# leabouffaut/DAS4Whales

Measured on AMD Instinct MI355X. Metric: channel-samples/sec through f-k filter + matched-filter, higher is better.
Workload: dtype f32 (matched filter: 2 x f16 split operands on the matrix cores, f32 accumulate); 1 GPU; 20000 channels x 120000 samples float32 per GPU, classic f-k fan mask (fk_filter_design defaults), stages fk+mf, HF+LF fin-call templates; api=public, parallelism=independent channel blocks x1

## Files before the change

das4whales_amd/csrc/xcorr_mm.hip:

```cpp
#include <cstdlib>

#include "mm_common.h"

namespace d4w {

#ifndef D4W_MM_CH
#define D4W_MM_CH 4096
#endif
constexpr int kMmCH = D4W_MM_CH;
constexpr int kMmKS = 6;
constexpr int kMmKSLong = 8;
constexpr int kMmKSMax = 16;
constexpr int kMmSection = 32 * kMmKSMax - 16;
constexpr int kMmMaxSupport = 32 * kMmKSLong - 15;
constexpr int kMmMaxSections = 16;
constexpr int kMmThreads = 256;
template <int KSM>
struct MmGeom {
    static constexpr int Halo = 32 * KSM;
    static constexpr int Stage = kMmCH + Halo;
    static constexpr int Q = (Stage + 4 * kMmThreads - 1) / (4 * kMmThreads);
    static constexpr int LastQ = (Stage - (Q - 1) * 4 * kMmThreads) / 4;
    static constexpr int Arr = Stage + 8;
};
__host__ __device__ constexpr int mm_pidx(int h) { return h; }

struct MmArgs {
    const float* x;
    const float* xnext;
    const double* mean;
    const float* maxabs;
    const float* taps;
    float* y0;
    float* y1;
    int nx, ns, ld_next, n_next, ltaps, len0, len1;
    float* rowmax0;
    float* rowmax1;
    int clamp;
    int shift;
    int accumulate;
    float tail0, tail1;
};

__device__ __forceinline__ float mm_wave_scan(float v) {
#ifdef D4W_EMU
    const int lane = (int)(threadIdx.x & 63);
    for (int off = 1; off < 64; off <<= 1) {
        const float n = __shfl_up(v, (unsigned)off);
        if (lane >= off) v += n;
    }
    return v;
#else
    auto dpp = [](float x, auto ctrl, auto rmask) {
        return __int_as_float(__builtin_amdgcn_update_dpp(0, __float_as_int(x), decltype(ctrl)::value, decltype(rmask)::value, 0xf, false));
    };
    v += dpp(v, std::integral_constant<int, 0x111>{}, std::integral_constant<int, 0xf>{});
    v += dpp(v, std::integral_constant<int, 0x112>{}, std::integral_constant<int, 0xf>{});
    v += dpp(v, std::integral_constant<int, 0x114>{}, std::integral_constant<int, 0xf>{});
    v += dpp(v, std::integral_constant<int, 0x118>{}, std::integral_constant<int, 0xf>{});
    v += dpp(v, std::integral_constant<int, 0x142>{}, std::integral_constant<int, 0xa>{});
    v += dpp(v, std::integral_constant<int, 0x143>{}, std::integral_constant<int, 0xc>{});
    return v;
#endif
}

template <int KS0, int KS1, int WPS, bool TAIL = false, bool WMAX = false, bool WSPLIT = false>
__global__ __launch_bounds__(kMmThreads, WPS) void xcorr_mm_rows(MmArgs P) {
    static_assert(!(WSPLIT && KS1 > 0), "the wave-split kernel is the one-template code run by two wave pairs");
    constexpr int KSM = KS0 > KS1 ? KS0 : KS1;
    using GEO = MmGeom<KSM>;
    constexpr int kMmHalo = GEO::Halo, kMmStage = GEO::Stage, kMmQ = GEO::Q, kMmLastQ = GEO::LastQ, kMmArr = GEO::Arr;
    constexpr int kSeg = 4 * kMmQ;
    D4W_DYN_LDS(smem_raw);
    mm_half* lds = reinterpret_cast<mm_half*>(smem_raw);
    float* red = reinterpret_cast<float*>(lds + 4 * kMmArr);
    constexpr int kBlk = kMmCH / 4;
    float* pb = red + 8;
    float* wt = pb + 2 * kBlk;
    const int tid = (int)threadIdx.x;
    const int lane = tid & 63, wv = mm_uniform(tid >> 6);
    const int n16 = lane & 15, g = lane >> 4;
    const int ns = P.ns;
    const int tsel = WSPLIT ? (wv >> 1) : 0;

    const int nchunk = (ns + kMmCH - 1) / kMmCH;
    const long long total = (long long)P.nx * nchunk;
    const int nparts = min(8, (int)gridDim.x);
    const int xcd = (int)blockIdx.x % nparts, wq = (int)blockIdx.x / nparts, nq = ((int)gridDim.x - xcd + nparts - 1) / nparts;
    const long long lo_c = total * xcd / nparts, hi_c = total * (xcd + 1) / nparts;
    mm_h8 a0h[KS0], a0l[KS0];
    mm_h8 a1h[KS1 ? KS1 : 1], a1l[KS1 ? KS1 : 1];
    float osc0 = 1.f, osc1 = 1.f;
#ifdef D4W_MM_V_TAIL_DEALT
    constexpr bool kRows = false;
#else
    constexpr bool kRows = TAIL;
#endif
    auto next_chunk = [&](long long c) -> long long {
        if constexpr (kRows) {
            const long long r = c / nchunk;
            return (c - r * nchunk + 1 < nchunk) ? c + 1 : (r + (long long)gridDim.x) * nchunk;
        } else {
            return c + nq;
        }
    };
    const long long end_c = kRows ? total : hi_c;
    long long c_n = kRows ? (long long)blockIdx.x * nchunk : lo_c + wq;
    {
        float* tl = reinterpret_cast<float*>(smem_raw);
        constexpr int TLP = 16 + kMmHalo;
        for (int i = tid; i < 2 * TLP; i += kMmThreads) {
            const int t = i / TLP, u = i - t * TLP - 15;
            const int L = t ? P.len1 : P.len0;
            float tv = (u >= 0 && u < L && (t == 0 || KS1 > 0 || WSPLIT)) ? P.taps[(size_t)t * P.ltaps + u] : 0.f;
            if constexpr (TAIL) {
                if (u < L && (t == 0 || KS1 > 0 || WSPLIT)) tv += t ? P.tail1 : P.tail0;
            }
            tl[i] = tv;
        }
        __syncthreads();
        auto build = [&](const float* tp, int L, auto& ah, auto& al, auto ks, float& osc) {
            constexpr int KS = decltype(ks)::value;
            float m = 0.f;
            for (int i = lane; i < TLP; i += 64) m = fmaxf(m, fabsf(tp[i]));
            for (int o = 32; o > 0; o >>= 1) m = fmaxf(m, __shfl_xor(m, o));
            float up, down;
            mm_pow2_scale(m, up, down);
            osc = up;
            (void)L;
            static_for<KS>([&](auto kq) {
                constexpr int kk = decltype(kq)::value;
                static_for<8>([&](auto jq) {
                    constexpr int j = decltype(jq)::value;
                    const float v = tp[15 + 32 * kk + 8 * g + j - n16] * down;
                    mm_half hi, lo;
                    mm_split(v, hi, lo);
                    mm_set(ah[kk], j, hi);
                    mm_set(al[kk], j, lo);
                });
            });
        };
        build(tl + (WSPLIT ? tsel * TLP : 0), WSPLIT && tsel ? P.len1 : P.len0, a0h, a0l, std::integral_constant<int, KS0>{}, osc0);
        if constexpr (KS1 > 0) build(tl + TLP, P.len1, a1h, a1l, std::integral_constant<int, KS1>{}, osc1);
        __syncthreads();
    }

    float4 pre[kMmQ];
    Mean2 mu_n{0.f, 0.f};
    float g_n = 1.f;
    bool heavy_n = false;
    bool tail_n = false;
    int row_n = 0, c0_n = 0;

    auto issue = [&](long long c) {
        row_n = (int)(c / nchunk);
        c0_n = (int)(c - (long long)row_n * nchunk) * kMmCH;
        mu_n = mean2_load(P.mean, row_n);
        g_n = 1.f;
        const int s0 = c0_n + P.shift;
        tail_n = s0 + kMmStage > ns;
        if (P.maxabs) {
            const float a = P.maxabs[row_n];
            g_n = (a > 0.f) ? 1.0f / a : 0.f;
            heavy_n = fabsf(mu_n.hi) > 0.9921875f * a;
        }
        const float* xr = P.x + (size_t)row_n * ns;
        const bool al = (reinterpret_cast<uintptr_t>(xr + s0) & 15) == 0;
        if (al && s0 + kMmStage <= ns) {
            const float4* p = reinterpret_cast<const float4*>(xr + s0) + tid;
            static_for<kMmQ>([&](auto qq) {
                constexpr int q = decltype(qq)::value;
                if (q < kMmQ - 1 || tid < kMmLastQ) pre[q] = mm_load4_stream(p + q * kMmThreads);
            });
        } else {
            if (al && (ns & 3) == 0) {
                static_for<kMmQ>([&](auto qq) {
                    constexpr int q = decltype(qq)::value;
                    if (q < kMmQ - 1 || tid < kMmLastQ) {
                        const int i = s0 + 4 * (tid + q * kMmThreads);
                        const float4 v = *reinterpret_cast<const float4*>(xr + min(i, ns - 4));
                        pre[q] = (i < ns) ? v : make_float4(mu_n.hi, mu_n.hi, mu_n.hi, mu_n.hi);
                    }
                });
            } else {
                static_for<kMmQ>([&](auto qq) {
                    constexpr int q = decltype(qq)::value;
                    if (q < kMmQ - 1 || tid < kMmLastQ) {
                        const int i = s0 + 4 * (tid + q * kMmThreads);
                        const float a0 = xr[min(i, ns - 1)], a1 = xr[min(i + 1, ns - 1)], a2 = xr[min(i + 2, ns - 1)], a3 = xr[min(i + 3, ns - 1)];
                        pre[q] = make_float4(i < ns ? a0 : mu_n.hi, i + 1 < ns ? a1 : mu_n.hi, i + 2 < ns ? a2 : mu_n.hi, i + 3 < ns ? a3 : mu_n.hi);
                    }
                });
            }
            if (P.xnext && P.n_next > 0 && s0 + kMmStage > ns) {
                const float* xn = P.xnext + (size_t)row_n * P.ld_next;
                const int n_next = P.n_next;
                static_for<kMmQ>([&](auto qq) {
                    constexpr int q = decltype(qq)::value;
                    if (q < kMmQ - 1 || tid < kMmLastQ) {
                        const int d = s0 + 4 * (tid + q * kMmThreads) - ns;
                        const float b0 = xn[min(max(d, 0), n_next - 1)], b1 = xn[min(max(d + 1, 0), n_next - 1)];
                        const float b2 = xn[min(max(d + 2, 0), n_next - 1)], b3 = xn[min(max(d + 3, 0), n_next - 1)];
                        if (d >= 0 && d < n_next) pre[q].x = b0;
                        if (d + 1 >= 0 && d + 1 < n_next) pre[q].y = b1;
                        if (d + 2 >= 0 && d + 2 < n_next) pre[q].z = b2;
                        if (d + 3 >= 0 && d + 3 < n_next) pre[q].w = b3;
                    }
                });
            }
        }
    };

    if (c_n < end_c) issue(c_n);
    int buf = 0;
    constexpr bool want_max = WMAX;
    float pst_hi = 0.f, pst_lo = 0.f;
    for (long long c = c_n; c < end_c;) {
        const int row = row_n, c0 = c0_n;
        const Mean2 mu = mu_n;
        const bool tail = tail_n;
        const int n_valid = ns + ((P.xnext && P.n_next > 0) ? P.n_next : 0) - c0 - P.shift;
        float gsc = g_n, osx = 1.f;
        const float gout = g_n;
        const bool own_scale = !P.maxabs || heavy_n;
        mm_half* bh = lds + (size_t)buf * 2 * kMmArr;
        mm_half* bl = bh + kMmArr;
        const long long c_next = next_chunk(c);
        const int cin = c0 / kMmCH;
        if (TAIL && cin == 0) { pst_hi = 0.f; pst_lo = 0.f; }
        const float pst = pst_hi;
        if (own_scale) {
            float m = 0.f;
            static_for<kMmQ>([&](auto qq) {
                constexpr int q = decltype(qq)::value;
                if (q < kMmQ - 1 || tid < kMmLastQ) {
                    const float4 v = pre[q];
                    const int at = 4 * (tid + q * kMmThreads);
                    float d0 = demean(v.x, mu), d1 = demean(v.y, mu), d2 = demean(v.z, mu), d3 = demean(v.w, mu);
                    if (tail) {
                        if (at >= n_valid) d0 = 0.f;
                        if (at + 1 >= n_valid) d1 = 0.f;
                        if (at + 2 >= n_valid) d2 = 0.f;
                        if (at + 3 >= n_valid) d3 = 0.f;
                    }
                    m = fmaxf(fmaxf(m, fmaxf(fabsf(d0), fabsf(d1))), fmaxf(fabsf(d2), fabsf(d3)));
                }
            });
            for (int o = 32; o > 0; o >>= 1) m = fmaxf(m, __shfl_xor(m, o));
            if (lane == 0) red[wv + 4 * buf] = m;
            lds_barrier();
            m = fmaxf(fmaxf(red[4 * buf], red[4 * buf + 1]), fmaxf(red[4 * buf + 2], red[4 * buf + 3]));
            mm_pow2_scale(m, osx, gsc);
        }
        const float mlg = -mu.lo * gsc;
        static_for<kMmQ>([&](auto qq) {
            constexpr int q = decltype(qq)::value;
            float s[4] = {0.f, 0.f, 0.f, 0.f};
            const bool mine = q < kMmQ - 1 || tid < kMmLastQ;
            const int at = mm_pidx(4 * (tid + q * kMmThreads));
            if (mine) {
                const float4 v = pre[q];
#ifdef D4W_MM_V_FLOATMEAN
                s[0] = (v.x - mu.hi) * gsc; s[1] = (v.y - mu.hi) * gsc; s[2] = (v.z - mu.hi) * gsc; s[3] = (v.w - mu.hi) * gsc;
#else
                s[0] = fmaf(v.x - mu.hi, gsc, mlg); s[1] = fmaf(v.y - mu.hi, gsc, mlg); s[2] = fmaf(v.z - mu.hi, gsc, mlg); s[3] = fmaf(v.w - mu.hi, gsc, mlg);
#endif
                if (P.clamp && !own_scale) static_for<4>([&](auto ee) { constexpr int e = decltype(ee)::value; s[e] = mm_clamp_half(s[e]); });
                if (tail) {
                    const int a0 = 4 * (tid + q * kMmThreads);
                    static_for<4>([&](auto ee) { constexpr int e = decltype(ee)::value; if (a0 + e >= n_valid) s[e] = 0.f; });
                }
#ifdef D4W_MM_V_OLDSPLIT
                mm_half h[4], l[4];
                static_for<4>([&](auto ee) { constexpr int e = decltype(ee)::value; mm_split(s[e], h[e], l[e]); });
                mm_put4(bh + at, h);
                mm_put4(bl + at, l);
#else
                mm_split_put4(s, bh + at, bl + at);
#endif
            }
#ifdef D4W_MM_V_TAIL_NOSCAN
            if constexpr (false) {
#else
            if constexpr (TAIL && q < kMmCH / (4 * kMmThreads)) {
#endif
                const float t4 = (s[0] + s[1]) + (s[2] + s[3]);
                const float inc = mm_wave_scan(t4);
                pb[buf * kBlk + kMmThreads * q + tid] = inc - t4;
                if (lane == 63) wt[buf * 16 + 4 * q + wv] = inc;
            }
        });
        if (c_next < end_c) issue(c_next);
        lds_barrier();
        float* ya = ((WSPLIT && tsel) ? P.y1 : P.y0) + (size_t)row * ns;
        float* yb = KS1 ? P.y1 + (size_t)row * ns : nullptr;
        const bool valign = ((reinterpret_cast<uintptr_t>(ya + c0) & 15) == 0) && (!KS1 || (reinterpret_cast<uintptr_t>(yb + c0) & 15) == 0);
        const float oxs = (own_scale && P.maxabs) ? osx * gout : osx;
        const float o0 = osc0 * oxs, o1 = osc1 * oxs;
        float segoff = 0.f;
        constexpr int NTW = kMmCH / 256 / (WSPLIT ? 2 : 4), NST = NTW * KSM, PF = 2;
        auto tile_of = [&](int ti) { return WSPLIT ? (wv & 1) + 2 * ti : wv + 4 * ti; };
        auto frag = [&](const mm_half* arr, int T, int kk) -> mm_h8 {
            const int gr = 32 * T + 2 * n16 + g + 4 * kk;
            return *reinterpret_cast<const mm_h8*>(arr + mm_pidx(8 * gr));
        };
        mm_h8 fh[PF + 1], fl[PF + 1];
        static_for<PF>([&](auto ss) {
            constexpr int s_ = decltype(ss)::value;
            fh[s_] = frag(bh, tile_of(s_ / KSM), s_ % KSM);
            fl[s_] = frag(bl, tile_of(s_ / KSM), s_ % KSM);
        });
        mm_f4 c0h = mm_zero(), c0l = mm_zero(), c1h = mm_zero(), c1l = mm_zero();
        float vmax0 = -INFINITY, vmax1 = -INFINITY;
        float vsum = 0.f;
        static_for<NST>([&](auto ss) {
            constexpr int s_ = decltype(ss)::value, ti = s_ / KSM, kk = s_ % KSM;
            if constexpr (s_ + PF < NST) {
                fh[(s_ + PF) % (PF + 1)] = frag(bh, tile_of((s_ + PF) / KSM), (s_ + PF) % KSM);
                fl[(s_ + PF) % (PF + 1)] = frag(bl, tile_of((s_ + PF) / KSM), (s_ + PF) % KSM);
            }
            mm_sched_fence();
            const mm_h8 xh = fh[s_ % (PF + 1)], xl = fl[s_ % (PF + 1)];
            if constexpr (kk < KS0) {
                c0h = mm_mfma(a0h[kk], xh, c0h);
                c0l = mm_mfma(a0h[kk], xl, c0l);
            }
            if constexpr (kk < KS1) {
                c1h = mm_mfma(a1h[kk], xh, c1h);
                c1l = mm_mfma(a1h[kk], xl, c1l);
            }
            if constexpr (kk < KS0) c0l = mm_mfma(a0l[kk], xh, c0l);
            if constexpr (kk < KS1) c1l = mm_mfma(a1l[kk], xh, c1l);
            mm_sched_fence();
            if constexpr (kk == KSM - 1) {
                const int T = tile_of(ti);
                const int kl = 256 * T + 16 * n16 + 4 * g;
                const int k = c0 + kl;
                if constexpr (ti == 0) {
                if constexpr (TAIL) {
                    const float w = lane < 16 ? wt[buf * 16 + lane] : 0.f;
                    const float inc = mm_wave_scan(w);
                    segoff = inc - w;
        #ifdef D4W_EMU
                    const float own = __shfl(inc, 15);
        #else
                    const float own = __builtin_bit_cast(float, __builtin_amdgcn_readlane(__builtin_bit_cast(int, inc), 15));
        #endif
                    const double pd = ((double)pst_hi + (double)pst_lo) + (double)(own * oxs);
                    const float ph = (float)pd, pl2 = (float)(pd - (double)ph);
        #ifdef D4W_EMU
                    pst_hi = ph; pst_lo = pl2;
        #else
                    pst_hi = __builtin_bit_cast(float, __builtin_amdgcn_readfirstlane(__builtin_bit_cast(int, ph)));
                    pst_lo = __builtin_bit_cast(float, __builtin_amdgcn_readfirstlane(__builtin_bit_cast(int, pl2)));
        #endif
                }
                }
                float r0[4], r1[4];
                float a0 = 0.f, a1 = 0.f;
#ifdef D4W_MM_V_TAIL_NOSCAN
                if constexpr (false) {
#else
                if constexpr (TAIL) {
#endif
#ifdef D4W_EMU
                    const float so = __shfl(segoff, T);
#else
                    const float so = __builtin_bit_cast(float, __builtin_amdgcn_readlane(__builtin_bit_cast(int, segoff), T));
#endif
                    const float pbk = fmaf(so + pb[buf * kBlk + kMmThreads * (T >> 2) + 64 * (T & 3) + 4 * n16], oxs, pst);
                    a0 = ((WSPLIT && tsel) ? P.tail1 : P.tail0) * pbk;
                    a1 = P.tail1 * pbk;
                }
                static_for<4>([&](auto rr) {
                    constexpr int r = decltype(rr)::value;
                    r0[r] = fmaf(fmaf(mm_get(c0l, r), kMmLoInv, mm_get(c0h, r)), o0, a0);
                    if constexpr (KS1 > 0) r1[r] = fmaf(fmaf(mm_get(c1l, r), kMmLoInv, mm_get(c1h, r)), o1, a1);
                });
                c0h = mm_zero(); c0l = mm_zero(); c1h = mm_zero(); c1l = mm_zero();
                if (valign && k + 3 < ns) {
                    if (KS1 == 0 && P.accumulate) {
                        const float4 o = mm_load4_stream(reinterpret_cast<const float4*>(ya + k));
                        r0[0] += o.x; r0[1] += o.y; r0[2] += o.z; r0[3] += o.w;
                    }
                    mm_store4(ya + k, r0[0], r0[1], r0[2], r0[3]);
                    if constexpr (KS1 > 0) mm_store4(yb + k, r1[0], r1[1], r1[2], r1[3]);
                    if (want_max) {
                        vmax0 = fmaxf(vmax0, fmaxf(fmaxf(r0[0], r0[1]), fmaxf(r0[2], r0[3])));
#ifndef D4W_MM_V_NONAN
                        vsum += (r0[0] + r0[1]) + (r0[2] + r0[3]);
#endif
                        if constexpr (KS1 > 0) {
                            vmax1 = fmaxf(vmax1, fmaxf(fmaxf(r1[0], r1[1]), fmaxf(r1[2], r1[3])));
#ifndef D4W_MM_V_NONAN
                            vsum += (r1[0] + r1[1]) + (r1[2] + r1[3]);
#endif
                        }
                    }
                } else {
                    for (int r = 0; r < 4; ++r)
                        if (k + r < ns) {
                            const float v0 = (KS1 == 0 && P.accumulate) ? ya[k + r] + r0[r] : r0[r];
                            ya[k + r] = v0;
                            if constexpr (KS1 > 0) yb[k + r] = r1[r];
                            if (want_max) {
                                vmax0 = fmaxf(vmax0, v0);
                                vsum += v0;
                                if constexpr (KS1 > 0) { vmax1 = fmaxf(vmax1, r1[r]); vsum += r1[r]; }
                            }
                        }
                }
            }
        });
        if (want_max) {
            for (int o = 32; o > 0; o >>= 1) {
                vmax0 = fmaxf(vmax0, __shfl_xor(vmax0, o));
                if constexpr (KS1 > 0) vmax1 = fmaxf(vmax1, __shfl_xor(vmax1, o));
            }
            const bool bad = __any(vsum != vsum);
            if (lane == 0) {
                mm_atomic_fmax(((WSPLIT && tsel) ? P.rowmax1 : P.rowmax0) + row, bad ? __uint_as_float(0x7FC00000u) : vmax0);
                if constexpr (KS1 > 0) mm_atomic_fmax(P.rowmax1 + row, bad ? __uint_as_float(0x7FC00000u) : vmax1);
            }
        }
        buf ^= 1;
        c = c_next;
    }
}

}

using namespace d4w;

extern "C" {

int d4w_xcorr_mm_max_support(void) { return kMmSection * kMmMaxSections; }

#define D4W_MM_LAUNCH(KS0, KS1, WPS, TAIL, grid, lds, stream, Q)                                                              \
    do {                                                                                                                      \
        if ((Q).rowmax0) D4W_LAUNCH((xcorr_mm_rows<KS0, KS1, WPS, TAIL, true>), dim3(grid), dim3(kMmThreads), lds, stream, Q);  \
        else D4W_LAUNCH((xcorr_mm_rows<KS0, KS1, WPS, TAIL, false>), dim3(grid), dim3(kMmThreads), lds, stream, Q);             \
    } while (0)

static int mm_one_template(MmArgs P, const float* taps, int len, float* y, float* rowmax, int grid, void* stream) {
    auto lds_of = [](int arr) { return (size_t)4 * arr * sizeof(mm_half) + 8 * sizeof(float); };
    const int nsec = (len <= 32 * kMmKSMax - 15) ? 1 : ceil_div(len, kMmSection);
    const int per = (nsec == 1) ? len : 16 * ceil_div(ceil_div(len, nsec), 16);
    for (int j = 0; j < nsec; ++j) {
        const int first = j * per;
        MmArgs Q = P;
        Q.taps = taps + first;
        Q.len0 = Q.len1 = std::min(per, len - first);
        Q.y0 = y;
        Q.y1 = nullptr;
        Q.shift = first;
        Q.accumulate = j > 0;
        Q.rowmax0 = (j == nsec - 1) ? rowmax : nullptr;
        Q.rowmax1 = nullptr;
        const int ks = ceil_div(Q.len0 + 15, 32);
        if (ks <= kMmKS)
            D4W_MM_LAUNCH(kMmKS, 0, 3, false, grid, lds_of(MmGeom<kMmKS>::Arr), stream, Q);
        else if (ks <= kMmKSLong)
            D4W_MM_LAUNCH(kMmKSLong, 0, 2, false, grid, lds_of(MmGeom<kMmKSLong>::Arr), stream, Q);
        else if (ks <= 12)
            D4W_MM_LAUNCH(12, 0, 2, false, grid, lds_of(MmGeom<12>::Arr), stream, Q);
        else
            D4W_MM_LAUNCH(kMmKSMax, 0, 2, false, grid, lds_of(MmGeom<kMmKSMax>::Arr), stream, Q);
    }
    return D4W_OK;
}

int d4w_xcorr_mm_f32(const float* x, int nx, int ns, const float* xnext, int ld_next, int n_next, const double* mean,
                     const float* maxabs, const float* taps, int ntpl, int ltaps, int len0, int len1, float* y0, float* y1,
                     void* stream) {
    return d4w_xcorr_mm_rowmax_f32(x, nx, ns, xnext, ld_next, n_next, mean, maxabs, taps, ntpl, ltaps, len0, len1, y0, y1, nullptr,
                                   nullptr, stream);
}

int d4w_xcorr_mm_rowmax_f32(const float* x, int nx, int ns, const float* xnext, int ld_next, int n_next, const double* mean,
                            const float* maxabs, const float* taps, int ntpl, int ltaps, int len0, int len1, float* y0, float* y1,
                            float* rowmax0, float* rowmax1, void* stream) {
    return d4w_xcorr_mm_tail_f32(x, nx, ns, xnext, ld_next, n_next, mean, maxabs, taps, ntpl, ltaps, len0, len1, 0.0, 0.0, y0, y1,
                                 rowmax0, rowmax1, stream);
}

int d4w_xcorr_mm_tail_max_support(void) { return 32 * kMmKSMax - 15; }

int d4w_xcorr_mm_tail_f32(const float* x, int nx, int ns, const float* xnext, int ld_next, int n_next, const double* mean,
                          const float* maxabs, const float* taps, int ntpl, int ltaps, int len0, int len1, double tail0, double tail1,
                          float* y0, float* y1, float* rowmax0, float* rowmax1, void* stream) {
    if (!x || !y0 || !taps || nx < 1 || ns < 1) return fail(D4W_EINVAL, "bad argument");
    if (ntpl == 2 && ((rowmax0 == nullptr) != (rowmax1 == nullptr))) return fail(D4W_EINVAL, "rowmax0 and rowmax1 go together");
    if (ntpl < 1 || ntpl > 2 || (ntpl == 2 && !y1)) return fail(D4W_EINVAL, "ntpl = %d (1 or 2 templates per call)", ntpl);
    if (xnext && (n_next < 0 || ld_next < n_next)) return fail(D4W_EINVAL, "a continuation needs 0 <= n_next <= ld_next");
    if (ntpl == 1) { len1 = len0; tail1 = 0.0; }
    if (len0 < 1 || len1 < 1 || len0 > ltaps || len1 > ltaps || std::max(len0, len1) > d4w_xcorr_mm_max_support())
        return fail(D4W_EINVAL, "template supports (%d, %d) must lie in 1..min(ltaps = %d, %d)", len0, len1, ltaps, d4w_xcorr_mm_max_support());
    const bool tails = tail0 != 0.0 || tail1 != 0.0;
    if (tails) {
        if (!mean || !maxabs) return fail(D4W_EINVAL, "the zero-padded template's tail needs the rows' statistics (mean, maxabs)");
        if (std::max(len0, len1) > d4w_xcorr_mm_tail_max_support())
            return fail(D4W_EINVAL, "with a tail the supports (%d, %d) must be <= %d", len0, len1, d4w_xcorr_mm_tail_max_support());
    }
    MmArgs P;
    P.x = x; P.xnext = xnext; P.mean = mean; P.maxabs = maxabs; P.taps = taps; P.y0 = y0; P.y1 = y1;
    P.nx = nx; P.ns = ns; P.ld_next = ld_next; P.n_next = xnext ? n_next : 0; P.ltaps = ltaps; P.len0 = len0; P.len1 = len1;
    P.shift = 0; P.accumulate = 0;
    static const int env_clamp = [] { const char* v = getenv("D4W_MM_CLAMP"); return v ? atoi(v) : 0; }();
    P.clamp = (xnext != nullptr && n_next > 0) || env_clamp;
    P.rowmax0 = rowmax0; P.rowmax1 = (ntpl == 2) ? rowmax1 : nullptr;
    P.tail0 = (float)tail0; P.tail1 = (float)tail1;
    if (rowmax0) {
        D4W_HIP(hipMemsetD32Async((hipDeviceptr_t)rowmax0, (int)0xFF800000u, (size_t)nx, (hipStream_t)stream));
        if (ntpl == 2) D4W_HIP(hipMemsetD32Async((hipDeviceptr_t)rowmax1, (int)0xFF800000u, (size_t)nx, (hipStream_t)stream));
    }
    const int nchunk = ceil_div(ns, kMmCH);
    const long long total = (long long)nx * nchunk;
    static const int env_wgs = [] { const char* v = getenv("D4W_MM_WGS"); const int n = v ? atoi(v) : 0; return n < 0 ? 0 : (n > 8 ? 8 : n); }();
    const int ks0 = ceil_div(len0 + 15, 32), ks1 = ceil_div(len1 + 15, 32);
    const bool fused = ntpl == 2 && std::max(ks0, ks1) <= kMmKS;
    const int per_cu = env_wgs ? env_wgs : ((ntpl == 1 && ks0 <= kMmKS) ? 3 : 2);
    const int ncu = mm_num_cus();
    const int grid = (int)std::min<long long>(total, (long long)ncu * per_cu);
    auto lds_of = [](int arr, bool tl) {
        return (size_t)4 * arr * sizeof(mm_half) + 8 * sizeof(float) + (tl ? ((size_t)2 * (kMmCH / 4) + 2 * 16) * sizeof(float) : 0);
    };
    static const int fused_form = [] { const char* v = getenv("D4W_MM_FUSED"); return v ? atoi(v) : 2; }();
    const int per_cu_ws = env_wgs ? env_wgs : 3;
#define D4W_MM_LAUNCH_WS(TAIL, grid, lds, Q)                                                                                            \
    do {                                                                                                                                \
        if ((Q).rowmax0) D4W_LAUNCH((xcorr_mm_rows<kMmKS, 0, 3, TAIL, true, true>), dim3(grid), dim3(kMmThreads), lds, stream, Q);       \
        else D4W_LAUNCH((xcorr_mm_rows<kMmKS, 0, 3, TAIL, false, true>), dim3(grid), dim3(kMmThreads), lds, stream, Q);                  \
    } while (0)
    if (tails) {
        const int grid_t = (int)std::min<long long>((long long)nx, (long long)ncu * per_cu);
        if (fused && fused_form != 2) {
            D4W_MM_LAUNCH_WS(true, (int)std::min<long long>((long long)nx, (long long)ncu * per_cu_ws), lds_of(MmGeom<kMmKS>::Arr, true), P);
            return D4W_OK;
        }
        if (fused) {
            const size_t lds = lds_of(MmGeom<kMmKS>::Arr, true);
            if (ks0 <= 5)
                D4W_MM_LAUNCH(5, kMmKS, 2, true, grid_t, lds, stream, P);
            else
                D4W_MM_LAUNCH(kMmKS, kMmKS, 2, true, grid_t, lds, stream, P);
            return D4W_OK;
        }
        for (int t = 0; t < ntpl; ++t) {
            MmArgs Q = P;
            Q.taps = taps + (size_t)t * ltaps;
            Q.len0 = Q.len1 = t ? len1 : len0;
            Q.tail0 = t ? (float)tail1 : (float)tail0;
            Q.tail1 = 0.f;
            Q.y0 = t ? y1 : y0;
            Q.y1 = nullptr;
            Q.rowmax0 = t ? rowmax1 : rowmax0;
            Q.rowmax1 = nullptr;
            const int ks = ceil_div(Q.len0 + 15, 32);
            if (ks <= kMmKS) {
                if (Q.rowmax0)
                    D4W_LAUNCH((xcorr_mm_rows<kMmKS, 0, 2, true, true>), dim3(grid_t), dim3(kMmThreads), lds_of(MmGeom<kMmKS>::Arr, true), stream, Q);
                else
                    D4W_LAUNCH((xcorr_mm_rows<kMmKS, 0, 3, true, false>), dim3(grid_t), dim3(kMmThreads), lds_of(MmGeom<kMmKS>::Arr, true), stream, Q);
            }
            else if (ks <= kMmKSLong)
                D4W_MM_LAUNCH(kMmKSLong, 0, 2, true, grid_t, lds_of(MmGeom<kMmKSLong>::Arr, true), stream, Q);
            else if (ks <= 12)
                D4W_MM_LAUNCH(12, 0, 2, true, grid_t, lds_of(MmGeom<12>::Arr, true), stream, Q);
            else
                D4W_MM_LAUNCH(kMmKSMax, 0, 2, true, grid_t, lds_of(MmGeom<kMmKSMax>::Arr, true), stream, Q);
        }
        return D4W_OK;
    }
    if (!fused) {
        int rc = mm_one_template(P, taps, len0, y0, rowmax0, grid, stream);
        if (rc == D4W_OK && ntpl == 2) rc = mm_one_template(P, taps + ltaps, len1, y1, rowmax1, grid, stream);
        return rc;
    }
    const size_t lds = lds_of(MmGeom<kMmKS>::Arr, false);
    if (fused_form != 2) {
        D4W_MM_LAUNCH_WS(false, (int)std::min<long long>(total, (long long)ncu * per_cu_ws), lds, P);
        return D4W_OK;
    }
    if (ks0 <= 5)
        D4W_MM_LAUNCH(5, kMmKS, 2, false, grid, lds, stream, P);
    else
        D4W_MM_LAUNCH(kMmKS, kMmKS, 2, false, grid, lds, stream, P);
    return D4W_OK;
}

}
```

Measured before the change: 119.1 billion channel-samples/s.

## Compute tail-correction prefix sums with MFMA ones-matrix and DPP row scans

Reworks the TAIL path's running-sum correction. It no longer does a full wave scan per float4 group and stores per-thread prefix values in LDS. Instead, each lane folds four group sums through quad-swap and row-shift DPP into 16-sample partials written to a small LDS table. The within-tile prefix is now obtained from an extra MFMA against a ones fragment plus a 16-lane row scan. This shrinks the LDS footprint and removes scattered LDS reads in the output epilogue, at the cost of one extra pair of MFMAs per tile and more DPP work.

```diff
diff --git a/das4whales_amd/csrc/xcorr_mm.hip b/das4whales_amd/csrc/xcorr_mm.hip
--- a/das4whales_amd/csrc/xcorr_mm.hip
+++ b/das4whales_amd/csrc/xcorr_mm.hip
@@ -42,6 +42,41 @@
     float tail0, tail1;
 };
 
+#ifndef D4W_EMU
+template <int CTRL, int RMASK = 0xf>
+__device__ __forceinline__ float mm_dpp(float v) {
+    return __int_as_float(__builtin_amdgcn_update_dpp(0, __float_as_int(v), CTRL, RMASK, 0xf, false));
+}
+#endif
+
+template <int N>
+__device__ __forceinline__ float mm_row_shr(float v) {
+#ifdef D4W_EMU
+    const float n = __shfl_up(v, (unsigned)N);
+    return ((int)(threadIdx.x & 15) >= N) ? n : 0.f;
+#else
+    return mm_dpp<0x110 + N>(v);
+#endif
+}
+
+template <int X>
+__device__ __forceinline__ float mm_quad_xor(float v) {
+    static_assert(X == 1 || X == 2, "a swap inside the quad");
+#ifdef D4W_EMU
+    return __shfl_xor(v, X);
+#else
+    return mm_dpp<X == 1 ? 0xB1 : 0x4E>(v);
+#endif
+}
+
+__device__ __forceinline__ float mm_row_scan(float v) {
+    v += mm_row_shr<1>(v);
+    v += mm_row_shr<2>(v);
+    v += mm_row_shr<4>(v);
+    v += mm_row_shr<8>(v);
+    return v;
+}
+
 __device__ __forceinline__ float mm_wave_scan(float v) {
 #ifdef D4W_EMU
     const int lane = (int)(threadIdx.x & 63);
@@ -51,16 +86,18 @@
     }
     return v;
 #else
-    auto dpp = [](float x, auto ctrl, auto rmask) {
-        return __int_as_float(__builtin_amdgcn_update_dpp(0, __float_as_int(x), decltype(ctrl)::value, decltype(rmask)::value, 0xf, false));
-    };
-    v += dpp(v, std::integral_constant<int, 0x111>{}, std::integral_constant<int, 0xf>{});
-    v += dpp(v, std::integral_constant<int, 0x112>{}, std::integral_constant<int, 0xf>{});
-    v += dpp(v, std::integral_constant<int, 0x114>{}, std::integral_constant<int, 0xf>{});
-    v += dpp(v, std::integral_constant<int, 0x118>{}, std::integral_constant<int, 0xf>{});
-    v += dpp(v, std::integral_constant<int, 0x142>{}, std::integral_constant<int, 0xa>{});
-    v += dpp(v, std::integral_constant<int, 0x143>{}, std::integral_constant<int, 0xc>{});
+    v = mm_row_scan(v);
+    v += mm_dpp<0x142, 0xa>(v);
+    v += mm_dpp<0x143, 0xc>(v);
     return v;
+#endif
+}
+
+__device__ __forceinline__ float mm_lane(float v, int L) {
+#ifdef D4W_EMU
+    return __shfl(v, L);
+#else
+    return __builtin_bit_cast(float, __builtin_amdgcn_readlane(__builtin_bit_cast(int, v), L));
 #endif
 }
 
@@ -74,9 +111,11 @@
     D4W_DYN_LDS(smem_raw);
     mm_half* lds = reinterpret_cast<mm_half*>(smem_raw);
     float* red = reinterpret_cast<float*>(lds + 4 * kMmArr);
-    constexpr int kBlk = kMmCH / 4;
-    float* pb = red + 8;
-    float* wt = pb + 2 * kBlk;
+    constexpr int kOwnQ = kMmCH / (4 * kMmThreads);
+    constexpr int kPart = kMmCH / 64;
+    constexpr int kPPL = kPart / 64;
+    static_assert(!TAIL || (kOwnQ % 4 == 0 && kPPL >= 1), "the tail's partial sums fold four loads into one value per lane");
+    float* wt = red + 8;
     const int tid = (int)threadIdx.x;
     const int lane = tid & 63, wv = mm_uniform(tid >> 6);
     const int n16 = lane & 15, g = lane >> 4;
@@ -95,6 +134,11 @@
     constexpr bool kRows = false;
 #else
     constexpr bool kRows = TAIL;
+#endif
+#ifdef D4W_MM_V_TAIL_NOSCAN
+    constexpr bool kTailSum = false;
+#else
+    constexpr bool kTailSum = TAIL;
 #endif
     auto next_chunk = [&](long long c) -> long long {
         if constexpr (kRows) {
@@ -144,6 +188,12 @@
         if constexpr (KS1 > 0) build(tl + TLP, P.len1, a1h, a1l, std::integral_constant<int, KS1>{}, osc1);
         __syncthreads();
     }
+    mm_h8 one_h, one_l;
+    static_for<8>([&](auto jq) {
+        constexpr int j = decltype(jq)::value;
+        mm_set(one_h, j, mm_to_half(g < 2 ? 1.f : 0.f));
+        mm_set(one_l, j, mm_to_half(g < 2 ? kMmLoInv : 0.f));
+    });
 
     float4 pre[kMmQ];
     Mean2 mu_n{0.f, 0.f};
@@ -253,6 +303,7 @@
             mm_pow2_scale(m, osx, gsc);
         }
         const float mlg = -mu.lo * gsc;
+        float t4[kOwnQ];
         static_for<kMmQ>([&](auto qq) {
             constexpr int q = decltype(qq)::value;
             float s[4] = {0.f, 0.f, 0.f, 0.f};
@@ -279,19 +330,24 @@
                 mm_split_put4(s, bh + at, bl + at);
 #endif
             }
-#ifdef D4W_MM_V_TAIL_NOSCAN
-            if constexpr (false) {
-#else
-            if constexpr (TAIL && q < kMmCH / (4 * kMmThreads)) {
-#endif
-                const float t4 = (s[0] + s[1]) + (s[2] + s[3]);
-                const float inc = mm_wave_scan(t4);
-                pb[buf * kBlk + kMmThreads * q + tid] = inc - t4;
-                if (lane == 63) wt[buf * 16 + 4 * q + wv] = inc;
-            }
+            if constexpr (kTailSum && q < kOwnQ) t4[q] = (s[0] + s[1]) + (s[2] + s[3]);
         });
+        if constexpr (kTailSum) {
+            const bool odd1 = (lane & 1) != 0, odd2 = (lane & 2) != 0;
+            static_for<kOwnQ / 4>([&](auto qg) {
+                constexpr int q0 = 4 * decltype(qg)::value;
+                const float m01 = (odd1 ? t4[q0 + 1] : t4[q0]) + mm_quad_xor<1>(odd1 ? t4[q0] : t4[q0 + 1]);
+                const float m23 = (odd1 ? t4[q0 + 3] : t4[q0 + 2]) + mm_quad_xor<1>(odd1 ? t4[q0 + 2] : t4[q0 + 3]);
+                float m = (odd2 ? m23 : m01) + mm_quad_xor<2>(odd2 ? m01 : m23);
+                m += mm_row_shr<4>(m);
+                m += mm_row_shr<8>(m);
+                if ((lane & 12) == 12) wt[buf * kPart + 16 * (q0 + (lane & 3)) + 4 * wv + g] = m;
+            });
+        }
         if (c_next < end_c) issue(c_next);
+#ifndef D4W_MM_V_NOHANDOFF
         lds_barrier();
+#endif
         float* ya = ((WSPLIT && tsel) ? P.y1 : P.y0) + (size_t)row * ns;
         float* yb = KS1 ? P.y1 + (size_t)row * ns : nullptr;
         const bool valign = ((reinterpret_cast<uintptr_t>(ya + c0) & 15) == 0) && (!KS1 || (reinterpret_cast<uintptr_t>(yb + c0) & 15) == 0);
@@ -311,6 +367,7 @@
             fl[s_] = frag(bl, tile_of(s_ / KSM), s_ % KSM);
         });
         mm_f4 c0h = mm_zero(), c0l = mm_zero(), c1h = mm_zero(), c1l = mm_zero();
+        mm_f4 cs = mm_zero();
         float vmax0 = -INFINITY, vmax1 = -INFINITY;
         float vsum = 0.f;
         static_for<NST>([&](auto ss) {
@@ -331,6 +388,7 @@
             }
             if constexpr (kk < KS0) c0l = mm_mfma(a0l[kk], xh, c0l);
             if constexpr (kk < KS1) c1l = mm_mfma(a1l[kk], xh, c1l);
+            if constexpr (kTailSum && kk == 0) cs = mm_mfma(one_l, xl, mm_mfma(one_h, xh, mm_zero()));
             mm_sched_fence();
             if constexpr (kk == KSM - 1) {
                 const int T = tile_of(ti);
@@ -338,14 +396,11 @@
                 const int k = c0 + kl;
                 if constexpr (ti == 0) {
                 if constexpr (TAIL) {
-                    const float w = lane < 16 ? wt[buf * 16 + lane] : 0.f;
+                    float w = 0.f;
+                    static_for<kPPL>([&](auto pp) { w += wt[buf * kPart + kPPL * lane + decltype(pp)::value]; });
                     const float inc = mm_wave_scan(w);
                     segoff = inc - w;
-        #ifdef D4W_EMU
-                    const float own = __shfl(inc, 15);
-        #else
-                    const float own = __builtin_bit_cast(float, __builtin_amdgcn_readlane(__builtin_bit_cast(int, inc), 15));
-        #endif
+                    const float own = mm_lane(inc, 63);
                     const double pd = ((double)pst_hi + (double)pst_lo) + (double)(own * oxs);
                     const float ph = (float)pd, pl2 = (float)(pd - (double)ph);
         #ifdef D4W_EMU
@@ -358,17 +413,10 @@
                 }
                 float r0[4], r1[4];
                 float a0 = 0.f, a1 = 0.f;
-#ifdef D4W_MM_V_TAIL_NOSCAN
-                if constexpr (false) {
-#else
-                if constexpr (TAIL) {
-#endif
-#ifdef D4W_EMU
-                    const float so = __shfl(segoff, T);
-#else
-                    const float so = __builtin_bit_cast(float, __builtin_amdgcn_readlane(__builtin_bit_cast(int, segoff), T));
-#endif
-                    const float pbk = fmaf(so + pb[buf * kBlk + kMmThreads * (T >> 2) + 64 * (T & 3) + 4 * n16], oxs, pst);
+                if constexpr (kTailSum) {
+                    const float so = mm_lane(segoff, 4 * T / kPPL);
+                    const float sa = mm_get(cs, 0);
+                    const float pbk = fmaf(so + (mm_row_scan(sa) - sa), oxs, pst);
                     a0 = ((WSPLIT && tsel) ? P.tail1 : P.tail0) * pbk;
                     a1 = P.tail1 * pbk;
                 }
@@ -523,7 +571,7 @@
     const int ncu = mm_num_cus();
     const int grid = (int)std::min<long long>(total, (long long)ncu * per_cu);
     auto lds_of = [](int arr, bool tl) {
-        return (size_t)4 * arr * sizeof(mm_half) + 8 * sizeof(float) + (tl ? ((size_t)2 * (kMmCH / 4) + 2 * 16) * sizeof(float) : 0);
+        return (size_t)4 * arr * sizeof(mm_half) + 8 * sizeof(float) + (tl ? (size_t)2 * (kMmCH / 64) * sizeof(float) : 0);
     };
     static const int fused_form = [] { const char* v = getenv("D4W_MM_FUSED"); return v ? atoi(v) : 2; }();
     const int per_cu_ws = env_wgs ? env_wgs : 3;
```

Measured after the change: 116.7 billion channel-samples/s. 2.0% lower.
